# Zhangwenyao1/DreamVLA

Hardware: AMD Instinct MI355X
Metric: train samples/sec (CALVIN ABC->D, seq_len=7) (higher is better)
Workload: dtype bf16; 1 GPU; DreamVLA CALVIN finetune step, head set C (obs_pred+depth_pred+sam_feat_pred+use_dit_head), B=32/GPU, S=7, window 10, 2x224^2 views, 77 text tokens, hidden 1024 / 24 layers / 16 heads, dropout 0.1 on, AdamW + clip 0.1; global_batch=32, seq_len=7, parallelism=dp1, grad_exchange=GradBucketReducer (flat bf16 buckets, async all-reduce), optimizer=FlatAdamW (HIP: dvla_sumsq_bf16 + dvla_adamw_bf16 on flat buffers)

## Files before the change

dreamvla_amd/_lib.py:

```python
import ctypes as C
import os

_HERE = os.path.dirname(os.path.abspath(__file__))
LIB_PATH = os.environ.get("DVLA_LIB") or os.path.join(_HERE, "libdvla_hip.so")

DT_BF16, DT_F32 = 0, 1
CROP_OUT_U8, CROP_OUT_BF16 = 0, 1
ABI_VERSION = 8
ACT = {"none": 0, "gelu": 1, "gelu_erf": 1, "gelu_tanh": 2, "gelu_new": 2, "relu": 3, "silu": 4,
       "quick_gelu": 5, "tanh": 6, "sigmoid": 7}

DVLA_ERRORS = {-1: "invalid argument", -2: "kernel launch failed", -3: "unsupported shape/alignment"}


class DvlaError(RuntimeError):
    pass


class GemmParams(C.Structure):
    _fields_ = [
        ("A", C.c_void_p), ("lda", C.c_int64), ("a_trans", C.c_int32),
        ("B", C.c_void_p), ("ldb", C.c_int64), ("b_trans", C.c_int32),
        ("C", C.c_void_p), ("ldc", C.c_int64), ("c_dtype", C.c_int32),
        ("M", C.c_int64), ("N", C.c_int64), ("K", C.c_int64),
# ... 62 lines not shown
    _fields_ = [("pred", C.c_void_p), ("pred_stride_n", C.c_int64), ("pred_stride_r", C.c_int64), ("row0", C.c_int32),
                ("patch", C.c_int32),
                ("imgs", C.c_void_p), ("imgs_dtype", C.c_int32), ("norm_pix", C.c_int32), ("H", C.c_int32), ("W", C.c_int32),
                ("mask", C.c_void_p), ("N", C.c_int64)]


_P, _I64, _I32, _F, _U32 = C.c_void_p, C.c_int64, C.c_int32, C.c_float, C.c_uint32
SYMBOLS = {
    "dvla_abi_version": (C.c_int, []),
    "dvla_gemm_bf16": (C.c_int, [C.POINTER(GemmParams), _P]),
    "dvla_gemm_ksum_partial_rows": (C.c_int64, [C.c_int32]),
    "dvla_set_gemm_variant": (None, [C.c_int]),
    "dvla_last_gemm_variant": (C.c_int, []),
    "dvla_set_gemm_schedule": (None, [C.c_int, C.c_int]),
    "dvla_get_gemm_schedule": (None, [C.POINTER(C.c_int), C.POINTER(C.c_int)]),
    "dvla_layernorm_fwd": (C.c_int, [_P, _P, _P, _I32, _P, _P, _P, _I64, _I64, _F, _P]),
    "dvla_layernorm_bwd": (C.c_int, [_P, _P, _P, _I32, _P, _P, _P, _P, _P, _P, _I64, _I64, _P]),
    "dvla_layernorm_bwd_add": (C.c_int, [_P, _P, _P, _I32, _P, _P, _P, _P, _P, _P, _I32, _P, _I64, _I64, _P]),
    "dvla_layernorm_bwd_partial_rows": (_I64, []),
    "dvla_layernorm_fwd_rows": (C.c_int, [_P, _P, _P, _I32, _P, _P, _P, _I64, _I64, _F, _I32, _I32, _I32, _I32, _P]),
    "dvla_layernorm_bwd_rows": (C.c_int, [_P, _P, _P, _I32, _P, _P, _P, _P, _P, _I32, _P, _I64, _I64, _I32, _I32, _I32, _I32, _P]),
    "dvla_attn_fwd": (C.c_int, [C.POINTER(AttnParams), _P]),
    "dvla_attn_bwd": (C.c_int, [C.POINTER(AttnParams), _P]),
    "dvla_attn_small_fwd": (C.c_int, [C.POINTER(AttnParams), _I32, _P]),
    "dvla_attn_small_bwd": (C.c_int, [C.POINTER(AttnParams), _I32, _P]),
    "dvla_attn_hd_fwd": (C.c_int, [C.POINTER(AttnParams), _I32, _P]),
    "dvla_attn_hd_bwd": (C.c_int, [C.POINTER(AttnParams), _I32, _P]),
    "dvla_colsum": (C.c_int, [_P, _I64, _I64, _I64, _P, _P, _P]),
    "dvla_colsum_dt": (C.c_int, [_P, _I64, _I64, _I64, _P, _I32, _P, _P]),
    "dvla_colsum_partial_rows": (_I64, []),
    "dvla_dropout": (C.c_int, [_P, _P, _I64, _I64, _F, _U32, _U32, _P]),
    "dvla_act_bwd": (C.c_int, [_P, _P, _P, _I64, _I64, _I32, _F, _U32, _U32, _P]),
    "dvla_act_bwd_colsum": (C.c_int, [_P, _P, _P, _I64, _I64, _I32, _F, _U32, _U32, _P, _I32, _P, _P]),
    "dvla_act_fwd": (C.c_int, [_P, _P, _I64, _I32, _P]),
    "dvla_ddim_cfg_step": (C.c_int, [_P, _I64, _P, _P, _I64, _I64, _F, _F, _F, _F, _F, _P]),
    "dvla_fm_cfg_step": (C.c_int, [_P, _I64, _P, _P, _I64, _I64, _F, _F, _P]),
    "dvla_dit_sample_workspace_bytes": (C.c_int64, [_I32]),
    "dvla_dit_sample": (C.c_int, [C.POINTER(DitSampleParams), _P]),
    "dvla_dit_sample_fm": (C.c_int, [C.POINTER(DitSampleParams), _P]),
    "dvla_dit_sample_set_stamps": (None, [_P]),
    "dvla_dit_sample_inject_timeouts": (None, [_I32]),
    "dvla_cast_f32_to_bf16": (C.c_int, [_P, _P, _I64, _P]),
    "dvla_cast_bf16_to_f32": (C.c_int, [_P, _P, _I64, _P]),
    "dvla_add": (C.c_int, [_P, _P, _P, _I64, _I64, _P]),
    "dvla_assemble_tokens": (C.c_int, [C.POINTER(TokenSrc), _I32, _P, _I64, _P, _I32, _I32, _I32, _I32, _P]),
    "dvla_mask_tables": (C.c_int, [C.POINTER(MaskRule), _P, _P, _P, _P, _P, _P]),
# ... 82 lines not shown
```

dreamvla_amd/csrc/attention.hip:

```cpp
#include "common.h"
#include "../../include/dvla.h"

namespace {

constexpr int AT_THREADS = 256;
constexpr int RM72 = 72;
constexpr int RM_BYTES = 32 * RM72 * 2;
constexpr int PI_BYTES = 16 * 64 * 4;
constexpr float LOG2E = 1.4426950408889634f;
constexpr float LN2 = 0.6931471805599453f;

struct AttnKArgs {
  const bf16_t *q, *k, *v; bf16_t* o;
  int64_t qsb, qst, qsh, ksb, kst, ksh, vsb, vst, vsh, osb, ost, osh;
  int B, H, Lq, Lk;
  float scale;
  const int32_t* key_index;
  const uint32_t *bits_q, *bits_k;
  const uint8_t* tile_map; int nqt, nkt;
  int has_drop; uint32_t drop_thr; float inv_keep; uint32_t seed_lo, seed_hi;
  float c1;
  float* lse;
  const bf16_t* dout; int64_t dsb, dst, dsh;
  float* delta;
  bf16_t *dq, *dk, *dv;
  int64_t dqsb, dqst, dqsh, dksb, dkst, dksh, dvsb, dvst, dvsh;
  int st16;
  int fuse_delta;
};

__device__ __forceinline__ int acc_row(int r, int g) { return (r & 3) + 8 * (r >> 2) + 4 * g; }

__device__ __forceinline__ uint4 load16(const bf16_t* p, bool ok) {
  return ok ? *reinterpret_cast<const uint4*>(p) : make_uint4(0u, 0u, 0u, 0u);
}

__device__ __forceinline__ void stage_rows_load(uint4 (&reg)[2], const bf16_t* base, int64_t stride, int row0, int nrows,
                                                const int32_t* index, int u) {
  const int pr = u >> 3, oct = u & 7;
#pragma unroll
  for (int e = 0; e < 2; ++e) {
    const int row = row0 + 2 * pr + e;
    const bool ok = row < nrows;
    const int src = (ok && index) ? index[row] : row;
    reg[e] = load16(base + (int64_t)src * stride + oct * 8, ok);
  }
}
__device__ __forceinline__ void stage_store_rm(const uint4 (&reg)[2], char* lds, int u) {
  const int pr = u >> 3, oct = u & 7;
  *reinterpret_cast<uint4*>(lds + ((2 * pr) * RM72 + oct * 8) * 2) = reg[0];
  *reinterpret_cast<uint4*>(lds + ((2 * pr + 1) * RM72 + oct * 8) * 2) = reg[1];
// ... 716 lines not shown
  a.osb = q->o_stride_b; a.ost = q->o_stride_t; a.osh = q->o_stride_h;
  a.B = q->B; a.H = q->H; a.Lq = q->Lq; a.Lk = q->Lk;
  a.scale = q->scale;
  a.key_index = q->key_index;
  a.bits_q = q->mask_bits_q; a.bits_k = q->mask_bits_k;
  a.tile_map = q->tile_map;
  a.nqt = (q->Lq + 31) / 32; a.nkt = (q->Lk + 31) / 32;
  a.has_drop = q->dropout_p > 0.f;
  a.inv_keep = a.has_drop ? 1.0f / (1.0f - q->dropout_p) : 1.0f;
  a.c1 = q->scale * a.inv_keep;
  {
    double thr = (double)q->dropout_p * 4294967296.0;
    a.drop_thr = thr >= 4294967295.0 ? 4294967295u : (uint32_t)thr;
  }
  a.seed_lo = q->seed_lo; a.seed_hi = q->seed_hi;
  a.lse = q->lse;
  a.dout = (const bf16_t*)q->dout; a.dsb = q->do_stride_b; a.dst = q->do_stride_t; a.dsh = q->do_stride_h;
  a.delta = q->delta;
  a.dq = (bf16_t*)q->dq; a.dk = (bf16_t*)q->dk; a.dv = (bf16_t*)q->dv;
  a.dqsb = q->dq_stride_b; a.dqst = q->dq_stride_t; a.dqsh = q->dq_stride_h;
  a.dksb = q->dk_stride_b; a.dkst = q->dk_stride_t; a.dksh = q->dk_stride_h;
  a.dvsb = q->dv_stride_b; a.dvst = q->dv_stride_t; a.dvsh = q->dv_stride_h;
  a.fuse_delta = 0;
  a.st16 = (ok16(q->o, q->o_stride_b, q->o_stride_t, q->o_stride_h) ? 1 : 0) |
           ((q->dq && ok16(q->dq, q->dq_stride_b, q->dq_stride_t, q->dq_stride_h)) ? 2 : 0) |
           ((q->dk && ok16(q->dk, q->dk_stride_b, q->dk_stride_t, q->dk_stride_h)) ? 4 : 0) |
           ((q->dv && ok16(q->dv, q->dv_stride_b, q->dv_stride_t, q->dv_stride_h)) ? 8 : 0);
  return DVLA_OK;
}

}

namespace {

__device__ __forceinline__ int fa_sw(int r) { return (((r >> 1) & 1) << 2) | ((r >> 2) & 3); }
__device__ __forceinline__ bf16x8 fa_frag_rm(const char* tile, int row, int s, int g) {
  return *reinterpret_cast<const bf16x8*>(tile + row * 128 + ((((2 * s + g) ^ fa_sw(row))) << 4));
}
__device__ __forceinline__ bf16x8 fa_frag_tr(const char* tile, int db, int mm, int lane) {
  const int gi = lane >> 4, c = lane & 15;
  const int d = 32 * db + 16 * (gi & 1) + 4 * (c & 3);
  union { fa_s16x4 h[2]; bf16x8 v; } u;
#pragma unroll
  for (int h = 0; h < 2; ++h) {
    const int row = 16 * mm + 8 * h + 4 * (gi >> 1) + (c >> 2);
    const int byte = row * 128 + ((((d >> 3) ^ fa_sw(row))) << 4) + (d & 7) * 2;
// ... 581 lines not shown
#pragma unroll
          for (int i = 0; i < 4; ++i) { td[i] = fa_frag_tr(dos, i >> 1, i & 1, lane); tq[i] = fa_frag_tr(qs, i >> 1, i & 1, lane); }
          fa_group4(td); fa_group4(tq);
          dvacc[0] = __builtin_amdgcn_mfma_f32_32x32x16_bf16(td[0], pf0, dvacc[0], 0, 0, 0);
          dkacc[0] = __builtin_amdgcn_mfma_f32_32x32x16_bf16(tq[0], sf0, dkacc[0], 0, 0, 0);
          dvacc[1] = __builtin_amdgcn_mfma_f32_32x32x16_bf16(td[2], pf0, dvacc[1], 0, 0, 0);
          dkacc[1] = __builtin_amdgcn_mfma_f32_32x32x16_bf16(tq[2], sf0, dkacc[1], 0, 0, 0);
          dvacc[0] = __builtin_amdgcn_mfma_f32_32x32x16_bf16(td[1], pf1, dvacc[0], 0, 0, 0);
          dkacc[0] = __builtin_amdgcn_mfma_f32_32x32x16_bf16(tq[1], sf1, dkacc[0], 0, 0, 0);
          dvacc[1] = __builtin_amdgcn_mfma_f32_32x32x16_bf16(td[3], pf1, dvacc[1], 0, 0, 0);
          dkacc[1] = __builtin_amdgcn_mfma_f32_32x32x16_bf16(tq[3], sf1, dkacc[1], 0, 0, 0);
        }
      }
      if (key_ok) {
        store_token(p.dk + (int64_t)b * p.dksb + (int64_t)key * p.dkst + (int64_t)h * p.dksh, dkacc, 1.0f, g, (p.st16 & 4) != 0);
        store_token(p.dv + (int64_t)b * p.dvsb + (int64_t)key * p.dvst + (int64_t)h * p.dvsh, dvacc, 1.0f, g, (p.st16 & 8) != 0);
      }
    }
    __syncthreads();
    if (next < n_items && (wave >> 2) == ((nt - 1) & 1)) issue_A_tile(next, nt - 1);
  }
}


__host__ __device__ inline size_t sf_smem_bytes(int nt) { return (size_t)nt * 2 * FA_TILE; }

__global__ __launch_bounds__(SB_THREADS) __attribute__((amdgpu_waves_per_eu(4, 4))) void attn_fwd_short_kernel(AttnKArgs p) {
  extern __shared__ __attribute__((aligned(16))) char smem[];
  const int t = threadIdx.x, lane = t & 63, l31 = lane & 31, g = lane >> 5;
  const int wave = __builtin_amdgcn_readfirstlane(t >> 6);
  const int L = p.Lq;
  const int nt = p.nqt;
  const int rounds = (nt + SB_WAVES - 1) / SB_WAVES;
  const float scale_log2 = p.scale * LOG2E;
  const uint32_t smem_base = (uint32_t)(uintptr_t)(__attribute__((address_space(3))) char*)smem;
  const int rl = 8 * (wave & 3) + (lane >> 3);
  const int oct = (lane & 7) ^ fa_sw(rl);
  const uint32_t kst2 = (uint32_t)p.kst * 2u, vst2 = (uint32_t)p.vst * 2u;
  auto issue_op = [&](const bf16_t* base, uint32_t stride_bytes, uint32_t region) {
    for (int tt = wave >> 2; tt < nt; tt += 2) {
      int row = tt * 32 + rl;
      row = row < L ? row : L - 1;
      const uint32_t dst = smem_base + region + (uint32_t)(tt * FA_TILE + (wave & 3) * 1024);
      fa_glds16(base, (uint32_t)row * stride_bytes + (uint32_t)(oct * 16), __builtin_amdgcn_readfirstlane(dst));
    }
  };
// ... 155 lines not shown
  if (smem <= 64 * 1024 && span_kv && !attn_force_staged())
#ifndef DVLA_ATTN_ABLATION
    hipLaunchKernelGGL(attn_fwd_ring_kernel<0>, ring_grid, block, smem, stream, a);
#else
    switch (attn_dbg()) {
      case 1: hipLaunchKernelGGL(attn_fwd_ring_kernel<1>, ring_grid, block, smem, stream, a); break;
      case 2: hipLaunchKernelGGL(attn_fwd_ring_kernel<2>, ring_grid, block, smem, stream, a); break;
      case 4: hipLaunchKernelGGL(attn_fwd_ring_kernel<4>, ring_grid, block, smem, stream, a); break;
      case 8: hipLaunchKernelGGL(attn_fwd_ring_kernel<8>, ring_grid, block, smem, stream, a); break;
      case 16: hipLaunchKernelGGL(attn_fwd_ring_kernel<16>, ring_grid, block, smem, stream, a); break;
      case 14: hipLaunchKernelGGL(attn_fwd_ring_kernel<14>, ring_grid, block, smem, stream, a); break;
      case 15: hipLaunchKernelGGL(attn_fwd_ring_kernel<15>, ring_grid, block, smem, stream, a); break;
      case 31: hipLaunchKernelGGL(attn_fwd_ring_kernel<31>, ring_grid, block, smem, stream, a); break;
      case 63: hipLaunchKernelGGL(attn_fwd_ring_kernel<63>, ring_grid, block, smem, stream, a); break;
      case 64: hipLaunchKernelGGL(attn_fwd_ring_kernel<64>, ring_grid, block, smem, stream, a); break;
      default: hipLaunchKernelGGL(attn_fwd_ring_kernel<0>, ring_grid, block, smem, stream, a); break;
    }
#endif
  else
    hipLaunchKernelGGL(attn_fwd_kernel, grid, block, 0, stream, a);
  return dvla_check_launch();
}

extern "C" int dvla_attn_bwd(const dvla_attn_params* q, void* stream_) {
  hipStream_t stream = reinterpret_cast<hipStream_t>(stream_);
  AttnKArgs a;
  int rc = fill_args(q, a);
  if (rc != DVLA_OK) return rc;
  if (!q->dout || !q->lse || !q->delta || !q->dq || !q->dk || !q->dv) return DVLA_ERR_ARG;
  if (q->tile_map && !q->mask_bits_k) return DVLA_ERR_ARG;
  if (!ok16(q->dout, q->do_stride_b, q->do_stride_t, q->do_stride_h)) return DVLA_ERR_UNSUPPORTED;
  auto ok8 = [](const void* ptr, int64_t s0, int64_t s1, int64_t s2) {
    return (reinterpret_cast<uintptr_t>(ptr) % 8 == 0) && (s0 % 4 == 0) && (s1 % 4 == 0) && (s2 % 4 == 0);
  };
  if (!ok8(q->dq, q->dq_stride_b, q->dq_stride_t, q->dq_stride_h) || !ok8(q->dk, q->dk_stride_b, q->dk_stride_t, q->dk_stride_h) ||
      !ok8(q->dv, q->dv_stride_b, q->dv_stride_t, q->dv_stride_h) || !ok16(q->o, q->o_stride_b, q->o_stride_t, q->o_stride_h))
    return DVLA_ERR_UNSUPPORTED;
  const int64_t nrows = (int64_t)a.B * a.H * a.Lq;
  dim3 block(AT_THREADS);
  const bool span_all = attn_span32(a.Lk, a.kst, false) && attn_span32(a.Lk, a.vst, false) && attn_span32(a.Lq, a.qst, false) &&
                        attn_span32(a.Lq, a.dst, false);
  if (attn_short_enabled() && !a.tile_map && !a.key_index && !a.has_drop && a.Lq == a.Lk && a.nqt <= SB_MAX_TILES && span_all &&
      !attn_force_staged()) {
    const size_t smem = sb_smem_bytes(a.nqt);
    static uint64_t attr_done = 0;
    int dev = 0;
    if (hipGetDevice(&dev) != hipSuccess || dev < 0 || dev >= 64) dev = 0;
    if (!(attr_done & (1ull << dev))) {
      (void)hipFuncSetAttribute(reinterpret_cast<const void*>(attn_bwd_short_kernel), hipFuncAttributeMaxDynamicSharedMemorySize, 160 * 1024);
      attr_done |= 1ull << dev;
    }
    int per_cu = (int)((size_t)(160 * 1024) / smem);
    if (per_cu < 1) per_cu = 1;
    if (per_cu > 2048 / SB_THREADS) per_cu = 2048 / SB_THREADS;
    const int64_t items = (int64_t)a.B * a.H;
    int64_t wgs = (int64_t)attn_num_cus() * per_cu;
    if (wgs > items) wgs = items;
    hipLaunchKernelGGL(attn_bwd_short_kernel, dim3((unsigned)wgs), dim3(SB_THREADS), smem, stream, a);
    return dvla_check_launch();
  }
  const size_t smem_dq = fa_smem_bytes(a.nkt, a.Lk, a.key_index != nullptr, a.tile_map != nullptr && a.bits_q != nullptr);
  const size_t smem_dkv = fa_dkv_smem_bytes(a.nqt, a.tile_map != nullptr && a.bits_k != nullptr, a.has_drop != 0);
  const dim3 grid_dq((unsigned)((a.nqt + 3) / 4), (unsigned)a.H, (unsigned)a.B);
  const dim3 grid_dkv((unsigned)((a.nkt + 3) / 4), (unsigned)a.H, (unsigned)a.B);
  const bool span_kv = attn_span32(a.Lk, a.kst, a.key_index != nullptr) && attn_span32(a.Lk, a.vst, a.key_index != nullptr);
  const bool span_q = attn_span32(a.Lq, a.qst, false) && attn_span32(a.Lq, a.dst, false);
  const bool dq_ring = smem_dq <= 64 * 1024 && span_kv && !attn_force_staged();
  a.fuse_delta = dq_ring ? 1 : 0;
  if (!dq_ring) {
    hipLaunchKernelGGL(attn_delta_kernel, dim3((unsigned)((nrows * 8 + 255) / 256)), dim3(256), 0, stream, a);
    rc = dvla_check_launch();
    if (rc != DVLA_OK) return rc;
  }
  if (dq_ring)
    hipLaunchKernelGGL(attn_bwd_dq_ring_kernel, grid_dq, block, smem_dq, stream, a);
  else
    hipLaunchKernelGGL(attn_bwd_dq_kernel, grid_dq, block, 0, stream, a);
  rc = dvla_check_launch();
  if (rc != DVLA_OK) return rc;
  if (smem_dkv <= 80 * 1024 && span_q && !attn_force_staged()) {
    if (smem_dkv > 64 * 1024) {
      static uint64_t attr_done = 0;
      int dev = 0;
      if (hipGetDevice(&dev) != hipSuccess || dev < 0 || dev >= 64) dev = 0;
      if (!(attr_done & (1ull << dev))) {
        (void)hipFuncSetAttribute(reinterpret_cast<const void*>(attn_bwd_dkv_ring_kernel), hipFuncAttributeMaxDynamicSharedMemorySize, 80 * 1024);
        attr_done |= 1ull << dev;
      }
    }
    hipLaunchKernelGGL(attn_bwd_dkv_ring_kernel, grid_dkv, block, smem_dkv, stream, a);
  }
  else
    hipLaunchKernelGGL(attn_bwd_dkv_kernel, grid_dkv, block, 0, stream, a);
  return dvla_check_launch();
}
```

dreamvla_amd/nn.py:

```python
import torch
from torch import nn

from . import ops


class Linear(nn.Linear):

    def forward(self, x, act="none", residual=None, dropout_p=0.0, ln_eps=None):
        if ln_eps is not None:
            return ops.linear_ln(x, self.weight, self.bias, eps=ln_eps, act=act, residual=residual)
        return ops.linear(x, self.weight, self.bias, act=act, residual=residual, dropout_p=dropout_p)


class LayerNorm(nn.LayerNorm):
    def forward(self, x):
        return ops.layer_norm(x, self.weight, self.bias, self.eps)

    def fork(self, x):
        return ops.layer_norm_fork(x, self.weight, self.bias, self.eps)

    def last_tokens(self, x, keep):
        return ops.layer_norm_last_tokens(x, self.weight, self.bias, self.eps, keep)


# ... 46 lines not shown

class Block(nn.Module):

    def __init__(self, dim, num_heads, mlp_ratio=4.0, qkv_bias=False, norm_layer=None, act="gelu_erf"):
        super().__init__()
        norm_layer = norm_layer or LayerNorm
        self.norm1 = norm_layer(dim)
        self.attn = Attention(dim, num_heads=num_heads, qkv_bias=qkv_bias)
        self.norm2 = norm_layer(dim)
        self.mlp = Mlp(in_features=dim, hidden_features=int(dim * mlp_ratio), act=act)

    def forward(self, x):
        if isinstance(self.norm1, LayerNorm) and isinstance(self.norm2, LayerNorm):
            r, n = self.norm1.fork(x)
            x = self.attn(n, residual=r)
            r, n = self.norm2.fork(x)
            return self.mlp(n, residual=r)
        x = self.attn(self.norm1(x), residual=x)
        x = self.mlp(self.norm2(x), residual=x)
        return x

    def forward_shared_suffix(self, prefix, suffix, n_seq):
        x = ops.concat_shared_suffix(prefix, suffix)
        qkv = ops.concat_shared_suffix(self.attn.qkv(self.norm1(prefix)), self.attn.qkv(self.norm1(suffix)))
        o = ops.self_attention(qkv, self.attn.num_heads, scale=self.attn.scale, head_dim=self.attn.head_dim)
        x = self.attn.proj(o, residual=x)
        r, n = self.norm2.fork(x)
        return self.mlp(n, residual=r)


class PatchEmbed(nn.Module):

    def __init__(self, img_size=224, patch_size=16, in_chans=3, embed_dim=768):
        super().__init__()
        self.img_size = (img_size, img_size)
        self.patch_size = (patch_size, patch_size)
        self.grid_size = (img_size // patch_size, img_size // patch_size)
        self.num_patches = self.grid_size[0] * self.grid_size[1]
        self.proj = nn.Conv2d(in_chans, embed_dim, kernel_size=patch_size, stride=patch_size)

    def forward(self, x, pos=None):
        n, c, hh, ww = x.shape
        p = self.patch_size[0]
        gh, gw = hh // p, ww // p
        cols = x.view(n, c, gh, p, gw, p).permute(0, 2, 4, 1, 3, 5).reshape(n * gh * gw, c * p * p)
        w = self.proj.weight.view(self.proj.weight.shape[0], -1)
        y = ops.linear(cols, w, self.proj.bias, residual=pos, res_rows=(gh * gw if pos is not None else 0))
        return y.view(n, gh * gw, -1)
# ... 1 lines not shown
```

dreamvla_amd/ops.py:

```python
import ctypes as C
import math
import os

import torch

from . import _lib
from ._lib import ACT, AttnParams, DT_BF16, DT_F32, GemmParams, check

BF16 = torch.bfloat16


def _stream():
    return torch.cuda.current_stream().cuda_stream


def _req(t, name, dtype=BF16):
    if not isinstance(t, torch.Tensor):
        raise TypeError(f"{name}: expected a tensor")
    if not t.is_cuda:
        raise _lib.DvlaError(f"{name}: tensor is on {t.device}; the DreamVLA HIP path has no CPU fallback")
    if dtype is not None and t.dtype != dtype:
        raise TypeError(f"{name}: expected {dtype}, got {t.dtype} (the kernels compute in bf16; fp32 parameters / activations "
                        f"are accepted by the module-level operators -- linear, mlp, layer_norm, attention -- which keep "
                        f"fp32 masters and run on bf16 shadows)")
# ... 1419 lines not shown
        srcs = (_lib.TokenSrc * 2)()
        srcs[0] = _lib.TokenSrc(prefix.data_ptr(), prefix.stride(0), 0, 0, nq)
        srcs[1] = _lib.TokenSrc(suffix.data_ptr(), 0, 0, nq, ns)
        out = torch.empty((n, nq + ns, D), dtype=BF16, device=prefix.device)
        check(lib.dvla_assemble_tokens(srcs, 2, None, D, out.data_ptr(), n, 1, nq + ns, D, _stream()), "dvla_assemble_tokens")
        ctx.nq, ctx.ns = nq, ns
        return out

    @staticmethod
    def backward(ctx, g):
        g = _req(g, "concat_shared_suffix.grad").contiguous()
        n, L, D = g.shape
        dp = g[:, :ctx.nq] if ctx.needs_input_grad[0] else None
        ds = None
        if ctx.needs_input_grad[1]:
            ds = colsum(g.view(n, L * D)[:, ctx.nq * D:], out_dtype=BF16).view(ctx.ns, D)
        return dp, ds


def concat_shared_suffix(prefix, suffix):
    return _ConcatSharedSuffix.apply(to_compute(prefix), to_compute(suffix))


def assemble_tokens(parts, pos=None):
    if len(parts) > 16:
        raise ValueError("assemble_tokens: at most 16 parts")
    return _AssembleTokens.apply(to_compute(pos), *[to_compute(t) for t in parts])


class _Dropout(torch.autograd.Function):
    @staticmethod
    def forward(ctx, x, p):
        _req(x, "dropout.input")
        seed = next_seed()
        ctx.p, ctx.seed, ctx.shape = p, seed, x.shape
        return dropout_raw(x.reshape(-1, x.shape[-1]), p, seed).view(x.shape)

    @staticmethod
    def backward(ctx, dy):
        return dropout_raw(dy.reshape(-1, ctx.shape[-1]), ctx.p, ctx.seed).view(ctx.shape), None


def dropout(x, p, training):
    if not training or p <= 0.0:
        return x
    return _Dropout.apply(to_compute(x), float(p))
# ... 310 lines not shown
```

include/dvla.h:

```cpp
#ifndef DVLA_H_
#define DVLA_H_
#include <stdint.h>
#ifdef __cplusplus
extern "C" {
#endif

#define DVLA_DT_BF16 0
#define DVLA_DT_F32 1

#define DVLA_ACT_NONE 0
#define DVLA_ACT_GELU_ERF 1
#define DVLA_ACT_GELU_TANH 2
#define DVLA_ACT_RELU 3
#define DVLA_ACT_SILU 4
#define DVLA_ACT_QUICK_GELU 5
#define DVLA_ACT_TANH 6
#define DVLA_ACT_SIGMOID 7

#define DVLA_ABI_VERSION 8
int dvla_abi_version(void);

typedef struct dvla_gemm_params {
  const void* A; int64_t lda; int32_t a_trans;
  const void* B; int64_t ldb; int32_t b_trans;
// ... 37 lines not shown
typedef struct dvla_attn_params {
  const void* q; const void* k; const void* v; void* o;
  int64_t q_stride_b, q_stride_t, q_stride_h;
  int64_t k_stride_b, k_stride_t, k_stride_h;
  int64_t v_stride_b, v_stride_t, v_stride_h;
  int64_t o_stride_b, o_stride_t, o_stride_h;
  int32_t B, H, Lq, Lk;
  float scale;
  const int32_t* key_index;
  const uint32_t* mask_bits_q;
  const uint32_t* mask_bits_k;
  const uint8_t* tile_map;
  float dropout_p; uint32_t seed_lo; uint32_t seed_hi;
  float* lse;
  const void* dout; int64_t do_stride_b, do_stride_t, do_stride_h;
  float* delta;
  void* dq; void* dk; void* dv;
  int64_t dq_stride_b, dq_stride_t, dq_stride_h;
  int64_t dk_stride_b, dk_stride_t, dk_stride_h;
  int64_t dv_stride_b, dv_stride_t, dv_stride_h;
} dvla_attn_params;
int dvla_attn_fwd(const dvla_attn_params* p, void* stream);
int dvla_attn_bwd(const dvla_attn_params* p, void* stream);
int dvla_attn_small_fwd(const dvla_attn_params* p, int32_t head_dim, void* stream);
int dvla_attn_small_bwd(const dvla_attn_params* p, int32_t head_dim, void* stream);
int dvla_attn_hd_fwd(const dvla_attn_params* p, int32_t head_dim, void* stream);
int dvla_attn_hd_bwd(const dvla_attn_params* p, int32_t head_dim, void* stream);

int dvla_colsum(const void* x, int64_t ld, int64_t rows, int64_t cols, float* out, float* partial, void* stream);
int dvla_colsum_dt(const void* x, int64_t ld, int64_t rows, int64_t cols, void* out, int32_t out_dtype, float* partial,
                   void* stream);
int64_t dvla_colsum_partial_rows(void);
int dvla_dropout(const void* x, void* y, int64_t rows, int64_t cols, float p, uint32_t seed_lo, uint32_t seed_hi,
                 void* stream);
int dvla_act_bwd(const void* dy, const void* preact, void* dz, int64_t rows, int64_t cols, int32_t act,
                 float dropout_p, uint32_t seed_lo, uint32_t seed_hi, void* stream);
int dvla_act_bwd_colsum(const void* dy, const void* preact, void* dz, int64_t rows, int64_t cols, int32_t act, float dropout_p,
                        uint32_t seed_lo, uint32_t seed_hi, void* colsum, int32_t colsum_dtype, float* partial, void* stream);
int dvla_act_fwd(const void* x, void* y, int64_t n, int32_t act, void* stream);
int dvla_ddim_cfg_step(const void* model_out, int64_t sample_stride, const float* x, float* x_next, int64_t bs, int64_t per_sample,
                       float cfg_scale, float a, float b, float sqrt_acp_prev, float sqrt_1m_acp_prev, void* stream);
int dvla_fm_cfg_step(const void* model_out, int64_t sample_stride, const float* x, float* x_next, int64_t bs, int64_t per_sample,
                     float cfg_scale, float delta, void* stream);
typedef struct dvla_dit_block_weights {
  const void *qkv_w, *qkv_b, *proj_w, *proj_b, *fc1_w, *fc1_b, *fc2_w, *fc2_b;
} dvla_dit_block_weights;
// ... 104 lines not shown
```

Before: 238.6 samples/s.

## Fuse shared-suffix gradient reduction into attention backward kernel

Adds a shared-suffix attention autograd op whose backward uses a new short-attention backward kernel. Each workgroup processes a fixed set of batch items per head and keeps running fp32 accumulators for the shared suffix rows' dQ/dK/dV in a workspace. A partial-row reduction then writes the suffix gradient directly, instead of writing full per-sample dQKV for suffix rows and column-summing it afterwards. This is meant to remove the full-size dQKV write for suffix tokens and the separate colsum pass. The cost is fp32 workspace traffic, extra global stores and loads of accumulators between items, and fewer workgroups (parts × H), which may lower occupancy.

```diff
diff --git a/dreamvla_amd/_lib.py b/dreamvla_amd/_lib.py
--- a/dreamvla_amd/_lib.py
+++ b/dreamvla_amd/_lib.py
@@ -108,6 +108,8 @@
     "dvla_layernorm_bwd_rows": (C.c_int, [_P, _P, _P, _I32, _P, _P, _P, _P, _P, _I32, _P, _I64, _I64, _I32, _I32, _I32, _I32, _P]),
     "dvla_attn_fwd": (C.c_int, [C.POINTER(AttnParams), _P]),
     "dvla_attn_bwd": (C.c_int, [C.POINTER(AttnParams), _P]),
+    "dvla_attn_bwd_shared_parts": (_I32, [C.POINTER(AttnParams), _I32, _I32]),
+    "dvla_attn_bwd_shared": (C.c_int, [C.POINTER(AttnParams), _I32, _I32, _P, _I64, _P, _P]),
     "dvla_attn_small_fwd": (C.c_int, [C.POINTER(AttnParams), _I32, _P]),
     "dvla_attn_small_bwd": (C.c_int, [C.POINTER(AttnParams), _I32, _P]),
     "dvla_attn_hd_fwd": (C.c_int, [C.POINTER(AttnParams), _I32, _P]),
diff --git a/dreamvla_amd/csrc/attention.hip b/dreamvla_amd/csrc/attention.hip
--- a/dreamvla_amd/csrc/attention.hip
+++ b/dreamvla_amd/csrc/attention.hip
@@ -27,6 +27,7 @@
   int64_t dqsb, dqst, dqsh, dksb, dkst, dksh, dvsb, dvst, dvsh;
   int st16;
   int fuse_delta;
+  int sh_row0; float* sh_ws;
 };
 
 __device__ __forceinline__ int acc_row(int r, int g) { return (r & 3) + 8 * (r >> 2) + 4 * g; }
@@ -789,6 +790,7 @@
   a.dksb = q->dk_stride_b; a.dkst = q->dk_stride_t; a.dksh = q->dk_stride_h;
   a.dvsb = q->dv_stride_b; a.dvst = q->dv_stride_t; a.dvsh = q->dv_stride_h;
   a.fuse_delta = 0;
+  a.sh_row0 = 0; a.sh_ws = nullptr;
   a.st16 = (ok16(q->o, q->o_stride_b, q->o_stride_t, q->o_stride_h) ? 1 : 0) |
            ((q->dq && ok16(q->dq, q->dq_stride_b, q->dq_stride_t, q->dq_stride_h)) ? 2 : 0) |
            ((q->dk && ok16(q->dk, q->dk_stride_b, q->dk_stride_t, q->dk_stride_h)) ? 4 : 0) |
@@ -1416,6 +1418,313 @@
   }
 }
 
+__device__ __forceinline__ int sb_opaque(int v) { asm volatile("" : "+v"(v)); return v; }
+__device__ __forceinline__ void sh_store(float* dst, const f32x16 (&acc)[2], int g) {
+#pragma unroll
+  for (int db = 0; db < 2; ++db)
+#pragma unroll
+    for (int rq = 0; rq < 4; ++rq)
+      *reinterpret_cast<float4*>(dst + 32 * db + 8 * rq + 4 * g) =
+          make_float4(acc[db][4 * rq], acc[db][4 * rq + 1], acc[db][4 * rq + 2], acc[db][4 * rq + 3]);
+}
+__device__ __forceinline__ void sh_load(const float* src, f32x16 (&acc)[2], int g) {
+#pragma unroll
+  for (int db = 0; db < 2; ++db)
+#pragma unroll
+    for (int rq = 0; rq < 4; ++rq) {
+      const float4 v = *reinterpret_cast<const float4*>(src + 32 * db + 8 * rq + 4 * g);
+      acc[db][4 * rq] = v.x; acc[db][4 * rq + 1] = v.y; acc[db][4 * rq + 2] = v.z; acc[db][4 * rq + 3] = v.w;
+    }
+}
+__device__ __forceinline__ void sh_store_run(float* dst, const f32x16 (&acc)[2]) {
+#pragma unroll
+  for (int i = 0; i < 8; ++i)
+    *reinterpret_cast<float4*>(dst + 256 * i) = make_float4(acc[i >> 2][4 * (i & 3)], acc[i >> 2][4 * (i & 3) + 1], acc[i >> 2][4 * (i & 3) + 2],
+                                                            acc[i >> 2][4 * (i & 3) + 3]);
+}
+__device__ __forceinline__ void sh_load_run(const float* src, f32x16 (&acc)[2]) {
+#pragma unroll
+  for (int i = 0; i < 8; ++i) {
+    const float4 v = *reinterpret_cast<const float4*>(src + 256 * i);
+    acc[i >> 2][4 * (i & 3)] = v.x; acc[i >> 2][4 * (i & 3) + 1] = v.y; acc[i >> 2][4 * (i & 3) + 2] = v.z; acc[i >> 2][4 * (i & 3) + 3] = v.w;
+  }
+}
+__global__ __launch_bounds__(SB_THREADS) void attn_bwd_short_shared_kernel(AttnKArgs p) {
+  extern __shared__ __attribute__((aligned(16))) char smem[];
+  const int t = threadIdx.x, lane = t & 63, l31 = lane & 31, g = lane >> 5;
+  const int wave = __builtin_amdgcn_readfirstlane(t >> 6);
+  const int L = p.Lq;
+  const int nt = p.nqt;
+  const int rounds = (nt + SB_WAVES - 1) / SB_WAVES;
+  const float scale_log2 = p.scale * LOG2E;
+
+  char* const regA = smem;
+  char* const regB = smem + (size_t)2 * nt * FA_TILE;
+  float* const lse2s = reinterpret_cast<float*>(smem + (size_t)4 * nt * FA_TILE);
+  float* const dlts = lse2s + 32 * nt;
+  const uint32_t smem_base = (uint32_t)(uintptr_t)(__attribute__((address_space(3))) char*)smem;
+  const uint32_t offA = 0u, offB = (uint32_t)(2 * nt * FA_TILE);
+
+  const int n_items = p.B * p.H;
+  const int lane0 = lane;
+  int lane_d = lane;
+  auto issue_op = [&](const bf16_t* base, uint32_t stride_bytes, uint32_t region) {
+    const int rl = 8 * (wave & 3) + (lane_d >> 3);
+    const int oct = (lane_d & 7) ^ fa_sw(rl);
+    for (int tt = wave >> 2; tt < nt; tt += 2) {
+      int row = tt * 32 + rl;
+      row = row < L ? row : L - 1;
+      const uint32_t dst = smem_base + region + (uint32_t)(tt * FA_TILE + (wave & 3) * 1024);
+      fa_glds16(base, (uint32_t)row * stride_bytes + (uint32_t)(oct * 16), __builtin_amdgcn_readfirstlane(dst));
+    }
+  };
+  const uint32_t qst2 = (uint32_t)p.qst * 2u, kst2 = (uint32_t)p.kst * 2u, vst2 = (uint32_t)p.vst * 2u, dst2 = (uint32_t)p.dst * 2u;
+  auto issue_A = [&](int item) {
+    const int b = item / p.H, h = item - b * p.H;
+    issue_op(p.q + (int64_t)b * p.qsb + (int64_t)h * p.qsh, qst2, offA);
+    issue_op(p.dout + (int64_t)b * p.dsb + (int64_t)h * p.dsh, dst2, offA + (uint32_t)(nt * FA_TILE));
+  };
+  auto issue_A_tile = [&](int item, int tt) {
+    const int b = item / p.H, h = item - b * p.H;
+    const int rl = 8 * (wave & 3) + (lane_d >> 3);
+    const int oct = (lane_d & 7) ^ fa_sw(rl);
+    int row = tt * 32 + rl;
+    row = row < L ? row : L - 1;
+    const uint32_t dst = smem_base + offA + (uint32_t)(tt * FA_TILE + (wave & 3) * 1024);
+    fa_glds16(p.q + (int64_t)b * p.qsb + (int64_t)h * p.qsh, (uint32_t)row * qst2 + (uint32_t)(oct * 16), __builtin_amdgcn_readfirstlane(dst));
+    fa_glds16(p.dout + (int64_t)b * p.dsb + (int64_t)h * p.dsh, (uint32_t)row * dst2 + (uint32_t)(oct * 16),
+              __builtin_amdgcn_readfirstlane(dst + (uint32_t)(nt * FA_TILE)));
+  };
+  auto issue_B = [&](int item) {
+    const int b = item / p.H, h = item - b * p.H;
+    issue_op(p.k + (int64_t)b * p.ksb + (int64_t)h * p.ksh, kst2, offB);
+    issue_op(p.v + (int64_t)b * p.vsb + (int64_t)h * p.vsh, vst2, offB + (uint32_t)(nt * FA_TILE));
+  };
+
+  int item = blockIdx.x;
+  if (item >= n_items) return;
+  issue_A(item);
+  issue_B(item);
+
+  uint4 ofr[4];
+  float lse_in = 0.f;
+  auto prefetch_o = [&](int it_) {
+    const int b_ = it_ / p.H, h_ = it_ - b_ * p.H;
+    const bf16_t* ob_ = p.o + (int64_t)b_ * p.osb + (int64_t)h_ * p.osh;
+    const int q = wave * 32 + (lane_d & 31);
+    const bool ok = wave < nt && q < L;
+#pragma unroll
+    for (int s = 0; s < 4; ++s) ofr[s] = load16(ob_ + (int64_t)q * p.ost + 16 * s + 8 * (lane_d >> 5), ok);
+    lse_in = ok ? p.lse[(b_ * p.H + h_) * L + q] : 0.f;
+  };
+  prefetch_o(item);
+
+  const int st0 = (p.sh_row0 + 31) / 32;
+  const int sh_w = 3 * p.H * 64;
+  float* const sh_part = p.sh_ws + (size_t)(blockIdx.x / (unsigned)p.H) * (size_t)((nt - st0) * 32) * sh_w + (blockIdx.x % (unsigned)p.H) * 64;
+  auto sh_rowp = [&](int j, int which, int row) { return sh_part + (size_t)((j - st0) * 32 + row) * sh_w + which * p.H * 64; };
+  float* const sh_run = p.sh_ws + (size_t)(gridDim.x / (unsigned)p.H) * (size_t)((nt - st0) * 32) * sh_w +
+                        (size_t)blockIdx.x * (size_t)((nt - st0) * 3 * 2048);
+  auto sh_runp = [&](int j, int which, int ln) { return sh_run + ((j - st0) * 3 + which) * 2048 + ln * 4; };
+  f32x16 dvacc[2] = {zero16(), zero16()};
+
+  for (; item < n_items; item += gridDim.x) {
+    const int b = item / p.H, h = item - b * p.H;
+    const int next = item + (int)gridDim.x;
+    const int row0 = (b * p.H + h) * L;
+    const bf16_t* ob = p.o + (int64_t)b * p.osb + (int64_t)h * p.osh;
+    const bool first_item = item == (int)blockIdx.x;
+
+    fa_wait_vmcnt<0>();
+#pragma unroll
+    for (int s = 0; s < 4; ++s) { fa_settle(ofr[s].x); fa_settle(ofr[s].y); fa_settle(ofr[s].z); fa_settle(ofr[s].w); }
+    fa_settle(lse_in);
+    __syncthreads();
+
+    {
+    const int lane = sb_opaque(lane0), l31 = lane & 31, g = lane >> 5;
+    for (int r = 0; r < rounds; ++r) {
+      const int j = wave + SB_WAVES * r;
+      if (j >= nt) break;
+      const bool shared = j >= st0;
+      const int q = j * 32 + l31;
+      const bool q_ok = q < L;
+      if (r > 0) {
+#pragma unroll
+        for (int s = 0; s < 4; ++s) ofr[s] = load16(ob + (int64_t)q * p.ost + 16 * s + 8 * g, q_ok);
+        lse_in = q_ok ? p.lse[row0 + q] : 0.f;
+      }
+      const char* qs = regA + (size_t)j * FA_TILE;
+      const char* dos = regA + (size_t)(nt + j) * FA_TILE;
+      bf16x8 qf[4], dof[4];
+#pragma unroll
+      for (int s = 0; s < 4; ++s) { qf[s] = fa_frag_rm(qs, l31, s, g); dof[s] = fa_frag_rm(dos, l31, s, g); }
+      float acc = 0.f;
+#pragma unroll
+      for (int s = 0; s < 4; ++s) {
+        const uint4 dv = *reinterpret_cast<const uint4*>(&dof[s]);
+        const uint32_t ow[4] = {ofr[s].x, ofr[s].y, ofr[s].z, ofr[s].w}, dw[4] = {dv.x, dv.y, dv.z, dv.w};
+#pragma unroll
+        for (int i = 0; i < 4; ++i) {
+          acc += bf2f((bf16_t)(dw[i] & 0xffff)) * bf2f((bf16_t)(ow[i] & 0xffff));
+          acc += bf2f((bf16_t)(dw[i] >> 16)) * bf2f((bf16_t)(ow[i] >> 16));
+        }
+      }
+      acc += __shfl_xor(acc, 32, 64);
+      const float lse2 = q_ok ? lse_in * LOG2E : INFINITY;
+      const float dlt = q_ok ? acc * p.scale : 0.f;
+      if (g == 0) { lse2s[j * 32 + l31] = lse2; dlts[j * 32 + l31] = dlt; }
+      f32x16 dqacc[2] = {zero16(), zero16()};
+      if (shared && !first_item) sh_load_run(sh_runp(j, 0, lane), dqacc);
+      for (int kt = 0; kt < nt; ++kt) {
+        const char* ks = regB + (size_t)kt * FA_TILE;
+        const char* vs = regB + (size_t)(nt + kt) * FA_TILE;
+        f32x16 sacc = zero16(), dpacc = zero16();
+        {
+          bf16x8 fk[4], fv[4];
+#pragma unroll
+          for (int s = 0; s < 4; ++s) { fk[s] = fa_frag_rm(ks, l31, s, g); fv[s] = fa_frag_rm(vs, l31, s, g); }
+          fa_group4(fk); fa_group4(fv);
+#pragma unroll
+          for (int s = 0; s < 4; ++s) {
+            sacc = __builtin_amdgcn_mfma_f32_32x32x16_bf16(fk[s], qf[s], sacc, 0, 0, 0);
+            dpacc = __builtin_amdgcn_mfma_f32_32x32x16_bf16(fv[s], dof[s], dpacc, 0, 0, 0);
+          }
+        }
+        const int k0 = kt * 32;
+        float ds[16];
+#pragma unroll
+        for (int rr = 0; rr < 16; ++rr) ds[rr] = fast_exp2(fmaf(sacc[rr], scale_log2, -lse2));
+        if (k0 + 32 > L) {
+          asm volatile("");
+          const uint32_t vg = low_mask(L - k0) >> (4 * g);
+          vis_select16<0u>(vg, ds);
+        }
+#pragma unroll
+        for (int rr = 0; rr < 16; ++rr) ds[rr] = ds[rr] * fmaf(dpacc[rr], p.scale, -dlt);
+        const bf16x8 f0 = pack_frag(ds), f1 = pack_frag(ds + 8);
+        bf16x8 kt4[4];
+#pragma unroll
+        for (int i = 0; i < 4; ++i) kt4[i] = fa_frag_tr(ks, i >> 1, i & 1, lane);
+        fa_group4(kt4);
+        dqacc[0] = __builtin_amdgcn_mfma_f32_32x32x16_bf16(kt4[0], f0, dqacc[0], 0, 0, 0);
+        dqacc[1] = __builtin_amdgcn_mfma_f32_32x32x16_bf16(kt4[2], f0, dqacc[1], 0, 0, 0);
+        dqacc[0] = __builtin_amdgcn_mfma_f32_32x32x16_bf16(kt4[1], f1, dqacc[0], 0, 0, 0);
+        dqacc[1] = __builtin_amdgcn_mfma_f32_32x32x16_bf16(kt4[3], f1, dqacc[1], 0, 0, 0);
+      }
+      if (shared) sh_store_run(sh_runp(j, 0, lane), dqacc);
+      else if (q_ok) store_token(p.dq + (int64_t)b * p.dqsb + (int64_t)q * p.dqst + (int64_t)h * p.dqsh, dqacc, 1.0f, g, (p.st16 & 2) != 0);
+    }
+    }
+    __syncthreads();
+    {
+    const int lane = sb_opaque(lane0), l31 = lane & 31, g = lane >> 5;
+
+    for (int r = rounds - 1; r >= 0; --r) {
+      const bool last_round = r == 0;
+      const int j = wave + SB_WAVES * r;
+      const bool active = j < nt;
+      const bool shared = active && j >= st0;
+      const int key = j * 32 + l31;
+      const bool key_ok = active && key < L;
+      bf16x8 kf[4], vf[4];
+      if (active) {
+        const char* ks = regB + (size_t)j * FA_TILE;
+        const char* vs = regB + (size_t)(nt + j) * FA_TILE;
+#pragma unroll
+        for (int s = 0; s < 4; ++s) { kf[s] = fa_frag_rm(ks, l31, s, g); vf[s] = fa_frag_rm(vs, l31, s, g); }
+      }
+      if (last_round) {
+        __syncthreads();
+        lane_d = sb_opaque(lane0);
+        if (next < n_items) { prefetch_o(next); issue_B(next); }
+      }
+      if (!active && !last_round) continue;
+      const bool parked = !last_round && wave >= st0;
+      if (parked) sh_store_run(sh_runp(wave, 2, lane), dvacc);
+      f32x16 dkacc[2] = {zero16(), zero16()};
+      if (shared && !first_item) sh_load_run(sh_runp(j, 1, lane), dkacc);
+      if (!(last_round && shared)) { dvacc[0] = zero16(); dvacc[1] = zero16(); }
+      if (!last_round && shared && !first_item) sh_load_run(sh_runp(j, 2, lane), dvacc);
+      for (int qt = 0; qt < nt; ++qt) {
+        const char* qs = regA + (size_t)qt * FA_TILE;
+        const char* dos = regA + (size_t)(nt + qt) * FA_TILE;
+        if (qt > 0 && last_round) {
+          __syncthreads();
+          if (next < n_items && (wave >> 2) == ((qt - 1) & 1)) issue_A_tile(next, qt - 1);
+        }
+        if (!active) continue;
+        f32x16 sacc = zero16(), dpacc = zero16();
+        {
+          bf16x8 fq[4], fd[4];
+#pragma unroll
+          for (int s = 0; s < 4; ++s) { fq[s] = fa_frag_rm(qs, l31, s, g); fd[s] = fa_frag_rm(dos, l31, s, g); }
+          fa_group4(fq); fa_group4(fd);
+#pragma unroll
+          for (int s = 0; s < 4; ++s) {
+            sacc = __builtin_amdgcn_mfma_f32_32x32x16_bf16(fq[s], kf[s], sacc, 0, 0, 0);
+            dpacc = __builtin_amdgcn_mfma_f32_32x32x16_bf16(fd[s], vf[s], dpacc, 0, 0, 0);
+          }
+        }
+        const int q0 = qt * 32;
+        float pr[16], ds[16];
+#pragma unroll
+        for (int rq = 0; rq < 4; ++rq) {
+          const float4 a = *reinterpret_cast<const float4*>(lse2s + q0 + 8 * rq + 4 * g);
+          const float4 c = *reinterpret_cast<const float4*>(dlts + q0 + 8 * rq + 4 * g);
+          const float l4[4] = {a.x, a.y, a.z, a.w}, d4[4] = {c.x, c.y, c.z, c.w};
+#pragma unroll
+          for (int e = 0; e < 4; ++e) {
+            const int rr = 4 * rq + e;
+            float pv = fast_exp2(fmaf(sacc[rr], scale_log2, -l4[e]));
+            pv = key_ok ? pv : 0.f;
+            pr[rr] = pv;
+            ds[rr] = pv * fmaf(dpacc[rr], p.scale, -d4[e]);
+          }
+        }
+        const bf16x8 pf0 = pack_frag(pr), pf1 = pack_frag(pr + 8);
+        const bf16x8 sf0 = pack_frag(ds), sf1 = pack_frag(ds + 8);
+        {
+          bf16x8 td[4], tq[4];
+#pragma unroll
+          for (int i = 0; i < 4; ++i) { td[i] = fa_frag_tr(dos, i >> 1, i & 1, lane); tq[i] = fa_frag_tr(qs, i >> 1, i & 1, lane); }
+          fa_group4(td); fa_group4(tq);
+          dvacc[0] = __builtin_amdgcn_mfma_f32_32x32x16_bf16(td[0], pf0, dvacc[0], 0, 0, 0);
+          dkacc[0] = __builtin_amdgcn_mfma_f32_32x32x16_bf16(tq[0], sf0, dkacc[0], 0, 0, 0);
+          dvacc[1] = __builtin_amdgcn_mfma_f32_32x32x16_bf16(td[2], pf0, dvacc[1], 0, 0, 0);
+          dkacc[1] = __builtin_amdgcn_mfma_f32_32x32x16_bf16(tq[2], sf0, dkacc[1], 0, 0, 0);
+          dvacc[0] = __builtin_amdgcn_mfma_f32_32x32x16_bf16(td[1], pf1, dvacc[0], 0, 0, 0);
+          dkacc[0] = __builtin_amdgcn_mfma_f32_32x32x16_bf16(tq[1], sf1, dkacc[0], 0, 0, 0);
+          dvacc[1] = __builtin_amdgcn_mfma_f32_32x32x16_bf16(td[3], pf1, dvacc[1], 0, 0, 0);
+          dkacc[1] = __builtin_amdgcn_mfma_f32_32x32x16_bf16(tq[3], sf1, dkacc[1], 0, 0, 0);
+        }
+      }
+      if (shared) {
+        sh_store_run(sh_runp(j, 1, lane), dkacc);
+        if (!last_round) sh_store_run(sh_runp(j, 2, lane), dvacc);
+      } else if (key_ok) {
+        store_token(p.dk + (int64_t)b * p.dksb + (int64_t)key * p.dkst + (int64_t)h * p.dksh, dkacc, 1.0f, g, (p.st16 & 4) != 0);
+        store_token(p.dv + (int64_t)b * p.dvsb + (int64_t)key * p.dvst + (int64_t)h * p.dvsh, dvacc, 1.0f, g, (p.st16 & 8) != 0);
+      }
+      if (parked) sh_load_run(sh_runp(wave, 2, lane), dvacc);
+    }
+    }
+    __syncthreads();
+    if (next < n_items && (wave >> 2) == ((nt - 1) & 1)) issue_A_tile(next, nt - 1);
+  }
+  for (int r = 0; r < rounds; ++r) {
+    const int j = wave + SB_WAVES * r;
+    if (j >= nt) break;
+    if (j < st0) continue;
+    if (r == 0) sh_store(sh_rowp(j, 2, l31), dvacc, g);
+    f32x16 a[2];
+    for (int which = 0; which < (r == 0 ? 2 : 3); ++which) {
+      sh_load_run(sh_runp(j, which, lane), a);
+      sh_store(sh_rowp(j, which, l31), a, g);
+    }
+  }
+}
+
 
 __host__ __device__ inline size_t sf_smem_bytes(int nt) { return (size_t)nt * 2 * FA_TILE; }
 
@@ -1617,8 +1926,31 @@
   return dvla_check_launch();
 }
 
-extern "C" int dvla_attn_bwd(const dvla_attn_params* q, void* stream_) {
-  hipStream_t stream = reinterpret_cast<hipStream_t>(stream_);
+static bool attn_bwd_short_ok(const AttnKArgs& a) {
+  const bool span_all = attn_span32(a.Lk, a.kst, false) && attn_span32(a.Lk, a.vst, false) && attn_span32(a.Lq, a.qst, false) &&
+                        attn_span32(a.Lq, a.dst, false);
+  return attn_short_enabled() && !a.tile_map && !a.key_index && !a.has_drop && a.Lq == a.Lk && a.nqt <= SB_MAX_TILES && span_all &&
+         !attn_force_staged();
+}
+static int64_t attn_bwd_short_wgs(const AttnKArgs& a) {
+  int per_cu = (int)((size_t)(160 * 1024) / sb_smem_bytes(a.nqt));
+  if (per_cu < 1) per_cu = 1;
+  if (per_cu > 2048 / SB_THREADS) per_cu = 2048 / SB_THREADS;
+  const int64_t items = (int64_t)a.B * a.H;
+  int64_t wgs = (int64_t)attn_num_cus() * per_cu;
+  if (wgs > items) wgs = items;
+  return wgs;
+}
+static int attn_bwd_shared_parts(const AttnKArgs& a, int first_shared_row, int max_workgroups) {
+  if (first_shared_row < 0 || first_shared_row >= a.Lq || !attn_bwd_short_ok(a)) return 0;
+  if ((first_shared_row + 31) / 32 >= a.nqt) return 0;
+  int64_t wgs = attn_bwd_short_wgs(a);
+  if (max_workgroups > 0 && wgs > max_workgroups) wgs = max_workgroups;
+  return (int)(wgs / a.H);
+}
+
+static int attn_bwd_launch(const dvla_attn_params* q, hipStream_t stream, int first_shared_row, int max_workgroups, float* sh_ws,
+                           int64_t sh_ws_floats, void* sh_out) {
   AttnKArgs a;
   int rc = fill_args(q, a);
   if (rc != DVLA_OK) return rc;
@@ -1633,25 +1965,29 @@
     return DVLA_ERR_UNSUPPORTED;
   const int64_t nrows = (int64_t)a.B * a.H * a.Lq;
   dim3 block(AT_THREADS);
-  const bool span_all = attn_span32(a.Lk, a.kst, false) && attn_span32(a.Lk, a.vst, false) && attn_span32(a.Lq, a.qst, false) &&
-                        attn_span32(a.Lq, a.dst, false);
-  if (attn_short_enabled() && !a.tile_map && !a.key_index && !a.has_drop && a.Lq == a.Lk && a.nqt <= SB_MAX_TILES && span_all &&
-      !attn_force_staged()) {
+  const int sh_parts = sh_ws ? attn_bwd_shared_parts(a, first_shared_row, max_workgroups) : 0;
+  if (sh_ws && sh_parts == 0) return DVLA_ERR_UNSUPPORTED;
+  if (attn_bwd_short_ok(a)) {
     const size_t smem = sb_smem_bytes(a.nqt);
     static uint64_t attr_done = 0;
     int dev = 0;
     if (hipGetDevice(&dev) != hipSuccess || dev < 0 || dev >= 64) dev = 0;
     if (!(attr_done & (1ull << dev))) {
       (void)hipFuncSetAttribute(reinterpret_cast<const void*>(attn_bwd_short_kernel), hipFuncAttributeMaxDynamicSharedMemorySize, 160 * 1024);
+      (void)hipFuncSetAttribute(reinterpret_cast<const void*>(attn_bwd_short_shared_kernel), hipFuncAttributeMaxDynamicSharedMemorySize, 160 * 1024);
       attr_done |= 1ull << dev;
     }
-    int per_cu = (int)((size_t)(160 * 1024) / smem);
-    if (per_cu < 1) per_cu = 1;
-    if (per_cu > 2048 / SB_THREADS) per_cu = 2048 / SB_THREADS;
-    const int64_t items = (int64_t)a.B * a.H;
-    int64_t wgs = (int64_t)attn_num_cus() * per_cu;
-    if (wgs > items) wgs = items;
-    hipLaunchKernelGGL(attn_bwd_short_kernel, dim3((unsigned)wgs), dim3(SB_THREADS), smem, stream, a);
+    if (sh_parts > 0) {
+      const int tile0 = (first_shared_row + 31) / 32;
+      const int64_t cols = (int64_t)(a.nqt - tile0) * 32 * 3 * a.H * 64;
+      if (!sh_out || sh_ws_floats < 2 * (int64_t)sh_parts * cols || reinterpret_cast<uintptr_t>(sh_ws) % 16 != 0) return DVLA_ERR_ARG;
+      a.sh_row0 = first_shared_row; a.sh_ws = sh_ws;
+      hipLaunchKernelGGL(attn_bwd_short_shared_kernel, dim3((unsigned)(sh_parts * a.H)), dim3(SB_THREADS), smem, stream, a);
+      rc = dvla_check_launch();
+      if (rc != DVLA_OK) return rc;
+      return dvla_reduce_partial_rows(sh_ws, sh_parts, cols, cols, sh_out, 1, stream);
+    }
+    hipLaunchKernelGGL(attn_bwd_short_kernel, dim3((unsigned)attn_bwd_short_wgs(a)), dim3(SB_THREADS), smem, stream, a);
     return dvla_check_launch();
   }
   const size_t smem_dq = fa_smem_bytes(a.nkt, a.Lk, a.key_index != nullptr, a.tile_map != nullptr && a.bits_q != nullptr);
@@ -1689,3 +2025,19 @@
     hipLaunchKernelGGL(attn_bwd_dkv_kernel, grid_dkv, block, 0, stream, a);
   return dvla_check_launch();
 }
+
+extern "C" int dvla_attn_bwd(const dvla_attn_params* q, void* stream_) {
+  return attn_bwd_launch(q, reinterpret_cast<hipStream_t>(stream_), 0, 0, nullptr, 0, nullptr);
+}
+
+extern "C" int32_t dvla_attn_bwd_shared_parts(const dvla_attn_params* q, int32_t first_shared_row, int32_t max_workgroups) {
+  AttnKArgs a;
+  if (fill_args(q, a) != DVLA_OK) return 0;
+  return attn_bwd_shared_parts(a, first_shared_row, max_workgroups);
+}
+
+extern "C" int dvla_attn_bwd_shared(const dvla_attn_params* q, int32_t first_shared_row, int32_t max_workgroups, float* workspace,
+                                    int64_t workspace_floats, void* d_shared, void* stream_) {
+  if (!workspace || !d_shared) return DVLA_ERR_ARG;
+  return attn_bwd_launch(q, reinterpret_cast<hipStream_t>(stream_), first_shared_row, max_workgroups, workspace, workspace_floats, d_shared);
+}
diff --git a/dreamvla_amd/nn.py b/dreamvla_amd/nn.py
--- a/dreamvla_amd/nn.py
+++ b/dreamvla_amd/nn.py
@@ -92,8 +92,8 @@
 
     def forward_shared_suffix(self, prefix, suffix, n_seq):
         x = ops.concat_shared_suffix(prefix, suffix)
-        qkv = ops.concat_shared_suffix(self.attn.qkv(self.norm1(prefix)), self.attn.qkv(self.norm1(suffix)))
-        o = ops.self_attention(qkv, self.attn.num_heads, scale=self.attn.scale, head_dim=self.attn.head_dim)
+        o = ops.attention_shared_suffix(self.attn.qkv(self.norm1(prefix)), self.attn.qkv(self.norm1(suffix)), self.attn.num_heads,
+                                        scale=self.attn.scale, head_dim=self.attn.head_dim)
         x = self.attn.proj(o, residual=x)
         r, n = self.norm2.fork(x)
         return self.mlp(n, residual=r)
diff --git a/dreamvla_amd/ops.py b/dreamvla_amd/ops.py
--- a/dreamvla_amd/ops.py
+++ b/dreamvla_amd/ops.py
@@ -1465,6 +1465,77 @@
     return _ConcatSharedSuffix.apply(to_compute(prefix), to_compute(suffix))
 
 
+ATTN_SHARED_BWD = os.environ.get("DVLA_ATTN_SHARED_BWD", "1") != "0"
+_ATTN_SHARED_MAX_WGS = 0
+
+
+class _AttentionSharedSuffix(torch.autograd.Function):
+
+    @staticmethod
+    def forward(ctx, prefix, suffix, H, scale):
+        lib = _lib.load()
+        _req(prefix, "attention_shared_suffix.prefix"); _req(suffix, "attention_shared_suffix.suffix")
+        n, nq, W = prefix.shape
+        ns = suffix.shape[0]
+        if suffix.shape[1] != W or W != 3 * H * 64:
+            raise ValueError("attention_shared_suffix: (n, nq, 3 * H * 64) and (ns, 3 * H * 64)")
+        if not (prefix.stride(2) == 1 and prefix.stride(1) == W and prefix.stride(0) % 8 == 0 and prefix.data_ptr() % 16 == 0):
+            prefix = prefix.contiguous()
+        suffix = suffix.contiguous()
+        L = nq + ns
+        srcs = (_lib.TokenSrc * 2)()
+        srcs[0] = _lib.TokenSrc(prefix.data_ptr(), prefix.stride(0), 0, 0, nq)
+        srcs[1] = _lib.TokenSrc(suffix.data_ptr(), 0, 0, nq, ns)
+        qkv = torch.empty((n, L, W), dtype=BF16, device=prefix.device)
+        check(lib.dvla_assemble_tokens(srcs, 2, None, W, qkv.data_ptr(), n, 1, L, W, _stream()), "dvla_assemble_tokens")
+        v5 = qkv.view(n, L, 3, H, 64)
+        need_grad = any(ctx.needs_input_grad)
+        o, lse = attn_fwd_raw(v5[:, :, 0], v5[:, :, 1], v5[:, :, 2], scale=scale, want_lse=need_grad)
+        ctx.H, ctx.scale, ctx.nq, ctx.ns = H, scale, nq, ns
+        if need_grad:
+            ctx.save_for_backward(qkv, o, lse)
+        return o.view(n, L, H * 64)
+
+    @staticmethod
+    def backward(ctx, dout):
+        lib = _lib.load()
+        qkv, o, lse = ctx.saved_tensors
+        n, L, W = qkv.shape
+        H, nq, ns = ctx.H, ctx.nq, ctx.ns
+        v5 = qkv.view(n, L, 3, H, 64)
+        do = _req(dout, "attention.grad_output").contiguous().view(n, L, H, 64)
+        p = _attn_params(v5[:, :, 0], v5[:, :, 1], v5[:, :, 2], o, H, L, ctx.scale, None, 0.0, (0, 0), lse)
+        parts = lib.dvla_attn_bwd_shared_parts(C.byref(p), nq, _ATTN_SHARED_MAX_WGS)
+        if parts == 0:
+            dqkv = torch.empty_like(qkv)
+            d5 = dqkv.view(n, L, 3, H, 64)
+            attn_bwd_raw(v5[:, :, 0], v5[:, :, 1], v5[:, :, 2], o, lse, do, d5[:, :, 0], d5[:, :, 1], d5[:, :, 2], scale=ctx.scale)
+            ds = colsum(dqkv.view(n, L * W)[:, nq * W:], out_dtype=BF16).view(ns, W) if ctx.needs_input_grad[1] else None
+            return dqkv[:, :nq], ds, None, None
+        tile0 = (nq + 31) // 32
+        keep = tile0 * 32
+        nrows = ((L + 31) // 32 - tile0) * 32
+        dqkv = torch.empty((n, keep, W), dtype=BF16, device=qkv.device)
+        d5 = dqkv.view(n, keep, 3, H, 64)
+        ds = torch.empty((keep - nq + nrows, W), dtype=BF16, device=qkv.device)
+        ws = torch.empty(2 * parts * nrows * W, dtype=torch.float32, device=qkv.device)
+        _attn_grad_params(p, do, d5[:, :, 0], d5[:, :, 1], d5[:, :, 2])
+        delta = torch.empty((n, H, L), dtype=torch.float32, device=qkv.device)
+        p.delta = delta.data_ptr()
+        check(lib.dvla_attn_bwd_shared(C.byref(p), nq, _ATTN_SHARED_MAX_WGS, ws.data_ptr(), ws.numel(), ds[keep - nq:].data_ptr(),
+                                       _stream()), "dvla_attn_bwd_shared")
+        if keep > nq:
+            colsum(dqkv.view(n, keep * W)[:, nq * W:], out_dtype=BF16, out=ds[:keep - nq].view(-1))
+        return dqkv[:, :nq], (ds[:ns] if ctx.needs_input_grad[1] else None), None, None
+
+
+def attention_shared_suffix(prefix_qkv, suffix_qkv, num_heads, *, scale=None, head_dim=64):
+    if head_dim != 64 or not ATTN_SHARED_BWD:
+        return self_attention(concat_shared_suffix(prefix_qkv, suffix_qkv), num_heads, scale=scale, head_dim=head_dim)
+    scale = (1.0 / math.sqrt(64.0)) if scale is None else scale
+    return _AttentionSharedSuffix.apply(to_compute(prefix_qkv), to_compute(suffix_qkv), int(num_heads), float(scale))
+
+
 def assemble_tokens(parts, pos=None):
     if len(parts) > 16:
         raise ValueError("assemble_tokens: at most 16 parts")
diff --git a/include/dvla.h b/include/dvla.h
--- a/include/dvla.h
+++ b/include/dvla.h
@@ -83,6 +83,9 @@
 } dvla_attn_params;
 int dvla_attn_fwd(const dvla_attn_params* p, void* stream);
 int dvla_attn_bwd(const dvla_attn_params* p, void* stream);
+int32_t dvla_attn_bwd_shared_parts(const dvla_attn_params* p, int32_t first_shared_row, int32_t max_workgroups);
+int dvla_attn_bwd_shared(const dvla_attn_params* p, int32_t first_shared_row, int32_t max_workgroups, float* workspace,
+                         int64_t workspace_floats, void* d_shared, void* stream);
 int dvla_attn_small_fwd(const dvla_attn_params* p, int32_t head_dim, void* stream);
 int dvla_attn_small_bwd(const dvla_attn_params* p, int32_t head_dim, void* stream);
 int dvla_attn_hd_fwd(const dvla_attn_params* p, int32_t head_dim, void* stream);
```

Result: no change. 238.3 samples/s (-0.1%).
